# ShuhongChen/panic3d-anime-reconstruction

Hardware: AMD Instinct MI355X
Metric: rendered rays/sec at 512^2 img x 96 samples/ray (higher is better)
Workload: dtype f32

## Files before the change

### panic3d-anime-reconstruction_amd/_build.py

```python
import os
import subprocess

HERE = os.path.dirname(os.path.abspath(__file__))
CSRC = os.path.join(HERE, "csrc")
SO = os.path.join(HERE, "libpanic3d_hip.so")
SOURCES = ["p3d_kernels.hip", "p3d_synthesis.hip", "p3d_conv_plain.hip", "p3d_conv_up.hip", "p3d_conv_up4.hip", "p3d_fir.hip", "p3d_torgb.hip",
           "p3d_mcubes.hip", "p3d_paste.hip", "p3d_render_grad.hip", "p3d_synthesis_grad.hip"]
HEADERS = ["p3d_math.hpp", "p3d_decode.hpp", "p3d_lds_layout.hpp", "p3d_render_plan.hpp", "p3d_conv_common.hpp", "p3d_conv_plan.hpp", "p3d_conv_stage.hpp", os.path.join("..", "..", "include", "panic3d_hip.h"),
           os.path.join("..", "..", "include", "p3d_numerics.h"), os.path.join("..", "..", "include", "p3d_mc_table.h"),
           "p3d_decode_grad.hpp", os.path.join("..", "..", "include", "p3d_render_grad.h"),
           os.path.join("..", "..", "include", "p3d_synthesis_grad.h")]
HIPCC_FLAGS = ["--offload-arch=gfx950", "-O3", "-std=c++17", "-ffp-contract=off", "-fno-fast-math", "-fno-slp-vectorize",
               "-mllvm", "-pragma-unroll-threshold=200000", "-fPIC", "-shared"]


def _hipcc():
    for c in (os.environ.get("HIPCC"), "/opt/rocm/bin/hipcc", "hipcc"):
        if c and (os.path.sep not in c or os.path.exists(c)):
            return c
    raise RuntimeError("hipcc not found")


def source_hash():
    import hashlib
    h = hashlib.sha256()
    for s in sorted(SOURCES + HEADERS):
        with open(os.path.join(CSRC, s), "rb") as f:
            h.update(s.encode() + b"\0" + f.read())
    return h.hexdigest()[:16]


RENDER_UNIT = ["p3d_kernels.hip", "p3d_decode.hpp", "p3d_lds_layout.hpp", "p3d_render_plan.hpp", "p3d_math.hpp", os.path.join("..", "..", "include", "panic3d_hip.h"),
               os.path.join("..", "..", "include", "p3d_numerics.h")]


def render_source_hash():
    import hashlib
    h = hashlib.sha256()
    for s in sorted(RENDER_UNIT):
        with open(os.path.join(CSRC, s), "rb") as f:
            h.update(s.encode() + b"\0" + f.read())
    return h.hexdigest()[:16]


SYNTHESIS_UNIT = ["p3d_synthesis.hip", "p3d_conv_plain.hip", "p3d_conv_up.hip", "p3d_conv_up4.hip", "p3d_fir.hip", "p3d_torgb.hip", "p3d_conv_common.hpp",
                  "p3d_conv_plan.hpp", "p3d_conv_stage.hpp", os.path.join("..", "..", "include", "panic3d_hip.h")]


def synthesis_source_hash():
    import hashlib
    h = hashlib.sha256()
    for s in sorted(SYNTHESIS_UNIT):
        with open(os.path.join(CSRC, s), "rb") as f:
            h.update(s.encode() + b"\0" + f.read())
    return h.hexdigest()[:16]


def built_hash(so=SO):
    import re
    try:
        with open(so, "rb") as f:
            m = re.search(rb"libpanic3d_hip gfx950[^\0]{0,64}src=([0-9a-f]{16})", f.read())
    except OSError:
        return None
    return m.group(1).decode() if m else None
# ... 86 lines not shown
```

### panic3d-anime-reconstruction_amd/csrc/p3d_kernels.hip

```cpp
#include <hip/hip_runtime.h>
#include <stddef.h>
#include <stdlib.h>
#include <string.h>

#include <atomic>
#include <type_traits>

#include "p3d_decode.hpp"
#include "p3d_render_plan.hpp"

#define P3D_WAVES_PER_WG 4
#define P3D_WG (64 * P3D_WAVES_PER_WG)

__global__ __launch_bounds__(256) void k_planes_to_nhwc(const float* __restrict__ src, float* __restrict__ dst, int HW) {
    __shared__ float tile[32][65];
    const int p0 = blockIdx.x * 64;
    const size_t img = (size_t)blockIdx.y * 32 * HW;
    {
        int px = threadIdx.x & 63, c0 = threadIdx.x >> 6;
#pragma unroll
        for (int k = 0; k < 8; ++k) {
            int c = c0 + 4 * k;
            tile[c][px] = (p0 + px < HW) ? src[img + (size_t)c * HW + p0 + px] : 0.0f;
        }
    }
    __syncthreads();
    {
        int c = threadIdx.x & 31, q0 = threadIdx.x >> 5;
#pragma unroll
        for (int k = 0; k < 8; ++k) {
            int px = q0 + 8 * k;
            if (p0 + px < HW) dst[img + (size_t)(p0 + px) * 32 + c] = tile[c][px];
        }
    }
}

struct DecodeParams {
    const float* planes;
    const float* coords;
    const float *w0, *b0, *w1, *b1;
    float* out_sigma;
    float* out_rgb;
// ... 203 lines not shown
    P3dDecodeCfg cfg;
};

struct MarchState {
    double Td;
    float W, D;
    float prev_t, prev_sigma;
};

P3D_DEV uint32_t p3d_fmix32(uint32_t h) {
    h ^= h >> 16; h *= 0x85EBCA6Bu; h ^= h >> 13; h *= 0xC2B2AE35u; h ^= h >> 16;
    return h;
}
P3D_DEV float p3d_draw(uint32_t seed_lo, uint32_t seed_hi, uint32_t stream, size_t ray, int idx) {
    uint32_t h = p3d_fmix32(seed_lo ^ ((uint32_t)ray * 0x9E3779B1u));
    h = p3d_fmix32(h ^ seed_hi ^ ((uint32_t)((unsigned long long)ray >> 32) * 0x7FEB352Du) ^ (((uint32_t)idx * 2u + stream) * 0x846CA68Bu));
    return (float)(h >> 8) * 0x1p-24f;
}

P3D_DEV float p3d_march_weight(MarchState& st, float t, float sigma, float& tm_out) {
    float dl = t - st.prev_t;
    float sm = (st.prev_sigma + sigma) * 0.5f;
    float tm = (st.prev_t + t) * 0.5f;
    float rho = p3d_softplus(sm - 1.0f);
    float dd = rho * dl;
    float alpha = 1.0f - p3d_exp(-dd);
    float T = (float)st.Td;
    float w = alpha * T;
    st.Td = st.Td * (double)((1.0f - alpha) + 1e-10f);
    tm_out = tm;
    return w;
}

P3D_DEV constexpr int p3d_pow2_ceil(int n) { int p = 1; while (p < n) p <<= 1; return p; }
template <int NR>
P3D_DEV void p3d_sort_network(float (&a)[NR]) {
    constexpr int N = p3d_pow2_ceil(NR);
#pragma unroll
    for (int pp = 1; pp < N; pp <<= 1) {
#pragma unroll
        for (int k = pp; k >= 1; k >>= 1) {
#pragma unroll
            for (int jj = k % pp; jj + k < N; jj += 2 * k) {
#pragma unroll
                for (int i = 0; i < k; ++i) {
                    if (i + jj + k < NR && (i + jj) / (2 * pp) == (i + jj + k) / (2 * pp)) {
                        float x = a[i + jj], y = a[i + jj + k];
                        a[i + jj] = __builtin_fminf(x, y);
                        a[i + jj + k] = __builtin_fmaxf(x, y);
                    }
                }
            }
        }
    }
}

template <int RS = 32>
P3D_DEV void p3d_lds_insertion_sort(float* A, int n, int j) {
    for (int i = 1; i < n; ++i) {
        float key = A[i * RS + j];
        int q = i - 1;
        while (q >= 0) {
            float v = A[q * RS + j];
            if (!(v > key)) break;
            A[(q + 1) * RS + j] = v;
            --q;
        }
        A[(q + 1) * RS + j] = key;
    }
}

template <int B, int RS, typename TCF>
P3D_DEV void p3d_inverse_cdf(const float* cdfA, TCF tc, int Ns, int j, const float (&ui)[B], float (&out)[B], int (&k_out)[B]) {
    const int n = Ns + 1;
    int pos[B];
#pragma unroll
    for (int q = 0; q < B; ++q) pos[q] = 0;
#pragma unroll
    for (int step = 128; step >= 1; step >>= 1) {
        if (step <= n) {
            float c[B];
#pragma unroll
            for (int q = 0; q < B; ++q) c[q] = cdfA[((pos[q] + step <= n) ? pos[q] + step - 1 : 0) * RS + j];
#pragma unroll
            for (int q = 0; q < B; ++q) pos[q] = ((pos[q] + step <= n) && (c[q] <= ui[q])) ? pos[q] + step : pos[q];
        }
    }
    float cb[B], ca[B], t0[B], t1[B], t2[B], t3[B];
#pragma unroll
    for (int q = 0; q < B; ++q) {
        const int k = pos[q], below = k - 1 > 0 ? k - 1 : 0, above = k < Ns ? k : Ns;
        k_out[q] = k;
        cb[q] = cdfA[below * RS + j]; ca[q] = cdfA[above * RS + j];
        t0[q] = tc(below); t1[q] = tc(below + 1);
        t2[q] = tc(above); t3[q] = tc(above + 1);
    }
#pragma unroll
    for (int q = 0; q < B; ++q) {
        float den = ca[q] - cb[q];
        if (den < 1e-5f) den = 1.0f;
        const float bb = 0.5f * (t0[q] + t1[q]), ba = 0.5f * (t2[q] + t3[q]);
        out[q] = bb + ((ui[q] - cb[q]) / den) * (ba - bb);
        asm volatile("" : "+v"(out[q]));
    }
}

#define P3D_NF_EXACT(NF) ((NF) == 48 || (NF) == 96)
template <int NF, bool DUMP, bool FAST, bool EARLY, bool TCG = p3d_render_tcg(NF, DUMP, EARLY)>
__global__ __launch_bounds__(64 * P3D_RENDER_WAVES, p3d_render_occ(NF, TCG)) void k_render(RenderParams p) {
    static_assert(!(DUMP && EARLY), "dumps need every sample decoded");
    static_assert(!TCG || p3d_render_tcg(NF, DUMP, EARLY), "TCG exists only for the production 96-key kernel");
    extern __shared__ __attribute__((aligned(16))) float lds[];
    p3d_load_mlp_to_lds(lds, p.w0, p.b0, p.w1, p.b1, !FAST);
    if constexpr (FAST) p3d_load_mlp_f16_to_lds(lds, p.w0, p.w1);
    __syncthreads();
    const int lane = threadIdx.x & 63, wave = threadIdx.x >> 6, j = lane & 31, h = lane >> 5;
    long long nblk = gridDim.x, b = blockIdx.x;
    const long long swz = p.swz;
    long long full = (nblk / (8 * swz)) * (8 * swz);
    long long bs = b;
    if (b < full) {
        long long slot = b >> 3, x = b & 7;
        const long long g = slot / swz, xr = p.blocked ? ((x + g) & 7) : x;
        bs = g * (8 * swz) + xr * swz + (slot % swz);
    }
    const int nwaves = blockDim.x >> 6;
    long long tile = bs * nwaves + wave;
    if (tile >= p.ntiles) return;
    float* wl = lds + (FAST ? P3D_LDS_FAST_FLOATS : P3D_LDS_MLP_FLOATS) + 4 + (size_t)wave * p.lds_rows * 32;

    const int Sc = p.Sc, Sf = P3D_NF_EXACT(NF) ? NF : p.Sf, S = Sc + Sf;
    long long n = tile / p.tiles_per_img, tl = tile - n * p.tiles_per_img;
    long long r;
    if (p.tile_w > 0) {
        long long ty = tl / p.tiles_x, tx = tl - ty * p.tiles_x;
        if (p.blocked) {
            const long long st = tl >> 8;
            const int q = (int)(tl & 255), SX = p.tiles_x >> 4;
            tx = (st % SX) * 16 + (q & 15);
            ty = (st / SX) * 16 + (q >> 4);
        }
        const int lx = (j & 1) | ((j >> 1) & 6), ly = ((j >> 1) & 1) | ((j >> 3) & 2);
        r = (ty * 4 + ly) * p.tile_w + tx * 8 + lx;
    } else {
        r = tl * 32 + j;
    }
    const bool active = r < p.R;
    const long long rc = active ? r : p.R - 1;
    const size_t ray = (size_t)n * p.R + rc;

    P3dPlaneGeom g;
    g.halfW = 0.5f * (float)p.W; g.halfH = 0.5f * (float)p.H; g.fW = (float)p.W; g.fH = (float)p.H; g.W = p.W;
    g.plane_bytes = (uint32_t)p.H * (uint32_t)p.W * 128u;
    unsigned nlo = __builtin_amdgcn_readfirstlane((unsigned)n);
    const float* pbase = p.planes + ((p.cfg.flags & P3D_FLAG_SHARED_PLANES) ? (size_t)0 : (size_t)nlo * 3 * (g.plane_bytes / 4));
    auto rs = __builtin_amdgcn_make_buffer_rsrc((void*)pbase, 0, 3 * g.plane_bytes, 0x00020000);
    const P3dDecodeCfg cfg = p.cfg;
    constexpr bool early = EARLY;
    const bool f_crop = (cfg.flags & P3D_FLAG_CROP) != 0;
    int ndec = 0;

// ... 55 lines not shown
        for (int i0 = 0; i0 < Sc; i0 += 8) {
            float jv[8];
#pragma unroll
            for (int q = 0; q < 8; ++q) {
                const int iq = i0 + q < Sc ? i0 + q : Sc - 1;
                jv[q] = p.rng ? p3d_draw(p.seed_lo, p.seed_hi, 0u, ray, iq) : jit[iq];
            }
#pragma unroll
            for (int q = 0; q < 8; ++q) {
                const int i = i0 + q;
                if (i < Sc) {
                    float lin = (i < Sc / 2) ? p3d_fma(step, (float)i, p.ray_start) : p3d_fma(-step, (float)(Sc - 1 - i), p.ray_end);
                    float t = lin + jv[q] * p.depth_delta;
                    if (limits) {
                        const float prod = ((float)i / (float)(Sc - 1)) * span;
                        t = (rs + prod) + jv[q] * rdelta;
                    } else if (p.disparity) {
                        const float s01 = 1.0f / (float)(Sc - 1);
                        const float l01 = (i < Sc / 2) ? p3d_fma(s01, (float)i, 0.0f) : p3d_fma(-s01, (float)(Sc - 1 - i), 1.0f);
                        const float dd = l01 + jv[q] * p.depth_delta;
                        const float ta_ = p.ray_start * (1.0f - dd), tb_ = p.ray_end * dd;
                        t = 1.0f / (ta_ + tb_);
                    }
                    tcA[i * 32 + j] = t;
                    unsorted |= (t < prev);
                    prev = t;
                    tcmin = __builtin_fminf(tcmin, t);
                    tcmax = __builtin_fmaxf(tcmax, t);
                    if constexpr (DUMP) if (dump && p.dumps.depths_coarse) p.dumps.depths_coarse[ray * Sc + i] = t;
                }
            }
        }
    }
    float tmin = __builtin_inff(), tmax = -__builtin_inff();
    if (Sf > 0) {
        MarchState st;
        st.Td = 1.0; st.W = 0.0f; st.D = 0.0f; st.prev_t = 0.0f; st.prev_sigma = 0.0f;
        uint32_t mword = 0;
        if constexpr (TCG) {
            float prev = -__builtin_inff(), pmax = -__builtin_inff();
            for (int i0 = 0; i0 < Sc; i0 += 8) {
                float jv[8];
#pragma unroll
                for (int q = 0; q < 8; ++q) jv[q] = jit_at(i0 + q < Sc ? i0 + q : Sc - 1);
#pragma unroll
                for (int q = 0; q < 8; ++q) {
                    const int i = i0 + q;
                    if (i >= Sc) break;
                    const float t = depth_of(i, jv[q]);
                    unsorted |= (t < prev);
                    bad_order |= (t < pmax);
                    pmax = __builtin_fmaxf(pmax, prev);
                    prev = t;
                    tcmin = __builtin_fminf(tcmin, t);
                    tcmax = __builtin_fmaxf(tcmax, t);
                    const float px = ox + t * dx, py = oy + t * dy, pz = oz + t * dz;
                    float sigma = P3D_SIGMA_MASKED;
                    const bool cropped = f_crop && (__builtin_fabsf(px) > cfg.crop_limit || __builtin_fabsf(pz) > cfg.crop_limit);
                    const bool live = !(cropped || st.Td < 1e-60);
                    const bool skip = __builtin_amdgcn_ballot_w64(live) == 0;
                    if (!skip) {
                        f32x16 dummy;
                        p3d_decode_wave<false, true>(lds, rs, g, cfg, px, py, pz, sigma, dummy, live);
                    }
                    mword |= (cropped || (live && sigma == P3D_SIGMA_MASKED)) ? (1u << (i & 31)) : 0u;
                    if ((i & 31) == 31 || i == Sc - 1) {
// ... 7 lines not shown
                    st.prev_t = t; st.prev_sigma = sigma;
                    ndec += skip ? 0 : 1;
                }
            }
        } else
        for (int i = 0; i < Sc; ++i) {
            float t = tcA[i * 32 + j];
            float px = ox + t * dx, py = oy + t * dy, pz = oz + t * dz;
            float sigma = P3D_SIGMA_MASKED;
            bool skip = false, live = true, cropped = false;
            if (early) {
                cropped = f_crop && (__builtin_fabsf(px) > cfg.crop_limit || __builtin_fabsf(pz) > cfg.crop_limit);
                live = !(cropped || st.Td < 1e-60);
                skip = __builtin_amdgcn_ballot_w64(live) == 0;
            }
            if (!skip) {
                f32x16 dummy;
                p3d_decode_wave<false, true>(lds, rs, g, cfg, px, py, pz, sigma, dummy, live);
            }
            if (early) {
                mword |= (cropped || (live && sigma == P3D_SIGMA_MASKED)) ? (1u << (i & 31)) : 0u;
                if ((i & 31) == 31 || i == Sc - 1) { mkA[(i >> 5) * 32 + j] = mword; mword = 0; }
            }
            if constexpr (DUMP) if (dump && p.dumps.sigma_coarse) p.dumps.sigma_coarse[ray * Sc + i] = sigma;
            if (i > 0) {
                float tm;
                float w = p3d_march_weight(st, t, sigma, tm);
                wcA[(i - 1) * 32 + j] = w;
                if constexpr (DUMP) if (dump && p.dumps.weights_coarse) p.dumps.weights_coarse[ray * (Sc - 1) + i - 1] = w;
            }
            st.prev_t = t; st.prev_sigma = sigma;
            if constexpr (!DUMP) ndec += skip ? 0 : 1;
        }
        const int Ns = Sc - 3;
        {
            double sum = 0.0;
            float wa = wcA[0 * 32 + j], wb = wcA[1 * 32 + j];
            for (int jj = 0; jj < Ns; ++jj) {
                float wc = wcA[(jj + 2) * 32 + j];
                float m1 = __builtin_fmaxf(wa, wb), m2 = __builtin_fmaxf(wb, wc);
                float v = ((m1 + m2) * 0.5f + 0.01f) + 1e-5f;
                sum += (double)v;
                wcA[(jj + 1) * 32 + j] = v;
                wa = wb; wb = wc;
            }
            float fsum = (float)sum;
            double acc = 0.0;
            wcA[j] = 0.0f;
            for (int jj = 0; jj < Ns; ++jj) {
                float pdf = wcA[(jj + 1) * 32 + j] / fsum;
                acc += (double)pdf;
                wcA[(jj + 1) * 32 + j] = (float)acc;
            }
        }
        const float* uu = p.u + ray * Sf;
        constexpr int DB = 8;
        if constexpr (NF > 0) {
            float tf[NF];
#pragma unroll
            for (int i = 0; i < NF; ++i)
                tf[i] = (i < Sf) ? (p.rng ? p3d_draw(p.seed_lo, p.seed_hi, 1u, ray, i) : uu[i]) : 0.0f;
#pragma unroll
            for (int i0 = 0; i0 < NF; i0 += DB) {
                if (i0 < Sf) {
                    float ub[DB], vb[DB];
                    int kb[DB];
#pragma unroll
                    for (int q = 0; q < DB; ++q) ub[q] = tf[i0 + q];
                    if constexpr (TCG) p3d_inverse_cdf<DB, 32>(wcA, tc_raw, Ns, j, ub, vb, kb);
                    else p3d_inverse_cdf<DB, 32>(wcA, tc_lds, Ns, j, ub, vb, kb);
#pragma unroll
                    for (int q = 0; q < DB; ++q) {
                        tf[i0 + q] = (i0 + q < Sf) ? vb[q] : __builtin_inff();
                        if constexpr (DUMP) {
                            if (dump && i0 + q < Sf && p.dumps.depths_fine) p.dumps.depths_fine[ray * Sf + i0 + q] = vb[q];
                            if (dump && i0 + q < Sf && p.dumps.inds) p.dumps.inds[ray * Sf + i0 + q] = kb[q];
                        }
                    }
                } else {
#pragma unroll
                    for (int q = 0; q < DB; ++q) tf[i0 + q] = __builtin_inff();
                }
            }
            p3d_sort_network<NF>(tf);
#pragma unroll
            for (int i = 0; i < NF; ++i)
                if (i < Sf) {
                    tfA[i * 32 + j] = tf[i];
                    if constexpr (TCG) {
                        const float px = ox + tf[i] * dx, pz = oz + tf[i] * dz;
                        const uint32_t b = (f_crop && (__builtin_fabsf(px) > cfg.crop_limit || __builtin_fabsf(pz) > cfg.crop_limit)) ? (1u << (i & 31)) : 0u;
                        if (i < 32) fw0 |= b; else if (i < 64) fw1 |= b; else fw2 |= b;
                    }
                }
        } else {
            for (int i0 = 0; i0 < Sf; i0 += DB) {
                float ub[DB], vb[DB];
                int kb[DB];
#pragma unroll
                for (int q = 0; q < DB; ++q) {
                    const int iq = i0 + q < Sf ? i0 + q : Sf - 1;
                    ub[q] = p.rng ? p3d_draw(p.seed_lo, p.seed_hi, 1u, ray, iq) : uu[iq];
                }
                p3d_inverse_cdf<DB, 32>(wcA, tc_lds, Ns, j, ub, vb, kb);
#pragma unroll
                for (int q = 0; q < DB; ++q) {
                    if (i0 + q < Sf) {
                        tfA[(i0 + q) * 32 + j] = vb[q];
                        if constexpr (DUMP) {
                            if (dump && p.dumps.depths_fine) p.dumps.depths_fine[ray * Sf + i0 + q] = vb[q];
                            if (dump && p.dumps.inds) p.dumps.inds[ray * Sf + i0 + q] = kb[q];
                        }
                    }
                }
            }
            p3d_lds_insertion_sort(tfA, Sf, j);
        }
        if constexpr (TCG) {
            wave_unsorted = __builtin_amdgcn_ballot_w64(unsorted) != 0;
            wave_bad = __builtin_amdgcn_ballot_w64(bad_order) != 0;
            if (wave_unsorted) { mw0 = 0u; mw1 = 0u; mw2 = 0u; }
        } else
        if (__builtin_amdgcn_ballot_w64(unsorted) != 0) {
            p3d_lds_insertion_sort(tcA, Sc, j);
            if (early) {
                for (int i = 0; i < ((Sc + 31) >> 5); ++i) mkA[i * 32 + j] = 0u;
            }
        }
    }
    MarchState st;
    st.Td = 1.0; st.W = 0.0f; st.D = 0.0f; st.prev_t = 0.0f; st.prev_sigma = 0.0f;
    f32x16 C, prev_rgb;
    float Cx = 0.0f, Cy = 0.0f, Cz = 0.0f;
#pragma unroll
    for (int c = 0; c < 16; ++c) { C[c] = 0.0f; prev_rgb[c] = 0.0f; }
    {
        int ci = 0, fi = 0;
        float ta = TCG ? 0.0f : tcA[j], tb = (Sf > 0) ? tfA[j] : __builtin_inff();
        tmin = __builtin_fminf(tcmin, tb);
        tmax = __builtin_fmaxf(tcmax, (Sf > 0) ? tfA[(Sf - 1) * 32 + j] : -__builtin_inff());
        bool prev_skipped = false, first = true, done = false;
        int m = 0;
        auto is_cropped = [&](float t) {
            const float px = ox + t * dx, pz = oz + t * dz;
            return f_crop && (__builtin_fabsf(px) > cfg.crop_limit || __builtin_fabsf(pz) > cfg.crop_limit);
        };
        auto advance = [&](bool take_c) {
            ci += take_c ? 1 : 0;
            fi += take_c ? 0 : 1;
            const int cq = ci < Sc ? ci : Sc - 1, fq = fi < Sf ? fi : (Sf > 0 ? Sf - 1 : 0);
            const float nv = (take_c ? tcA : tfA)[(take_c ? cq : fq) * 32 + j];
            ta = take_c ? nv : ta;
            tb = take_c ? tb : nv;
        };
        float tcn = 0.0f;
        if constexpr (TCG) {
            uint32_t slw[6], knw[6];
#pragma unroll
            for (int w = 0; w < 6; ++w) { slw[w] = 0u; knw[w] = 0u; }
            for (int i0 = 0; i0 < Sc; i0 += 8) {
                float tv[8];
                int pos[8];
#pragma unroll
                for (int q = 0; q < 8; ++q) { tv[q] = tc_sorted(i0 + q < Sc ? i0 + q : Sc - 1); pos[q] = 0; }
#pragma unroll
                for (int step = 64; step >= 1; step >>= 1) {
                    float c[8];
#pragma unroll
                    for (int q = 0; q < 8; ++q) c[q] = tfA[((pos[q] + step <= Sf) ? pos[q] + step - 1 : 0) * 32 + j];
#pragma unroll
                    for (int q = 0; q < 8; ++q) pos[q] = ((pos[q] + step <= Sf) && (c[q] < tv[q])) ? pos[q] + step : pos[q];
                }
#pragma unroll
                for (int q = 0; q < 8; ++q) {
                    const int i = i0 + q;
                    if (i >= Sc) break;
                    const uint32_t mwv = (i < 32) ? mw0 : (i < 64 ? mw1 : mw2);
                    const bool known = is_cropped(tv[q]) || ((mwv >> (i & 31)) & 1u);
                    const int P = i + pos[q], pw = P >> 5;
                    const uint32_t b = 1u << (P & 31);
#pragma unroll
                    for (int w = 0; w < 6; ++w) {
                        slw[w] |= (pw == w) ? b : 0u;
                        knw[w] |= (pw == w && known) ? b : 0u;
                    }
                }
            }
            if (__builtin_amdgcn_ballot_w64((fw0 | fw1 | fw2) != 0u) != 0) {
                int fk = 0;
#pragma unroll
                for (int w = 0; w < 6; ++w) {
                    if (w * 32 < S) {
                        uint32_t kk = 0u;
                        for (int b = 0; b < 32; ++b) {
                            const bool isf = !((slw[w] >> b) & 1u) && (w * 32 + b < S);
                            const uint32_t fwv = (fk < 32) ? fw0 : (fk < 64 ? fw1 : fw2);
                            kk |= (isf && ((fwv >> (fk & 31)) & 1u)) ? (1u << b) : 0u;
                            fk += isf ? 1 : 0;
                        }
                        knw[w] |= kk;
                    }
                }
            }
#pragma unroll
            for (int w = 0; w < 6; ++w)
                if (w < nmw) { knA[w * 32 + j] = knw[w]; slA[w * 32 + j] = slw[w]; }
            tcn = tc_sorted(0);
        } else
        if constexpr (EARLY) {
            uint32_t kw = 0u, sw = 0u;
            for (int q = 0; q < S; ++q) {
                const bool take_c = (ci < Sc) && (fi >= Sf || ta <= tb);
                bool known = is_cropped(take_c ? ta : tb);
                if (take_c && Sf > 0) known = known || ((mkA[(ci >> 5) * 32 + j] >> (ci & 31)) & 1u);
                kw |= known ? (1u << (q & 31)) : 0u;
                sw |= take_c ? (1u << (q & 31)) : 0u;
                advance(take_c);
                if ((q & 31) == 31 || q == S - 1) {
                    knA[(q >> 5) * 32 + j] = kw; slA[(q >> 5) * 32 + j] = sw;
                    kw = 0u; sw = 0u;
                }
            }
            ci = 0;
        }
        for (int it = 0;; ++it) {
            bool take_c, known = false;
            float t;
            if constexpr (!EARLY) {
                if (it >= S) break;
                take_c = (ci < Sc) && (fi >= Sf || ta <= tb);
                t = take_c ? ta : tb;
                advance(take_c);
            } else {
                if (!done && st.Td < (FAST ? 2e-6 : 1e-60)) done = true;
                if (!done && (first || st.prev_sigma <= 602.0f)) {
                    bool any = false, last_c = false;
                    while (m < S) {
                        const int sh = m & 31, left = (32 - sh < S - m) ? 32 - sh : S - m;
                        const uint32_t kw = knA[(m >> 5) * 32 + j] >> sh, sw = slA[(m >> 5) * 32 + j] >> sh;
                        int run = (~kw != 0u) ? __builtin_ctz(~kw) : 32;
                        run = run < left ? run : left;
                        if (run > 0) {
                            const uint32_t inrun = run >= 32 ? 0xffffffffu : ((1u << run) - 1u);
                            ci += __builtin_popcount(sw & inrun);
                            last_c = (sw >> (run - 1)) & 1u;
                            any = true;
                            m += run;
                        }
                        if (run < left) break;
                    }
                    if (any) {
                        if constexpr (TCG) {
                            const float pc = tc_sorted(ci > 0 ? ci - 1 : 0);
                            tcn = tc_sorted(ci < Sc ? ci : Sc - 1);
                            st.prev_t = last_c ? pc : tfA[(m - ci - 1 > 0 ? m - ci - 1 : 0) * 32 + j];
                        } else
                        st.prev_t = last_c ? tcA[(ci - 1) * 32 + j] : tfA[(m - ci - 1) * 32 + j];
                        st.prev_sigma = P3D_SIGMA_MASKED;
                        prev_skipped = true; first = false;
                    }
                    done = m >= S;
                }
                if (__builtin_amdgcn_ballot_w64(!done) == 0) break;
                const int mm = done ? S - 1 : m;
                const uint32_t kb = knA[(mm >> 5) * 32 + j] >> (mm & 31), sb = slA[(mm >> 5) * 32 + j] >> (mm & 31);
                take_c = (sb & 1u) != 0u;
                known = !done && (kb & 1u) != 0u;
                const int cq = ci < Sc ? ci : Sc - 1, fq = (m - ci < Sf) ? m - ci : (Sf > 0 ? Sf - 1 : 0);
                if constexpr (TCG) t = take_c ? tcn : tfA[fq * 32 + j];
                else t = (take_c || Sf == 0) ? tcA[cq * 32 + j] : tfA[fq * 32 + j];
                if (!done) { ++m; ci += take_c ? 1 : 0; }
                if constexpr (TCG) {
                    if (!done && take_c) tcn = tc_sorted(ci < Sc ? ci : Sc - 1);
                }
            }
            const bool have = EARLY ? !done : true;
            const float px = ox + t * dx, py = oy + t * dy, pz = oz + t * dz;
            float sigma = P3D_SIGMA_MASKED;
            f32x16 rgb;
#pragma unroll
            for (int c = 0; c < 16; ++c) rgb[c] = 0.0f;
            const bool live = have && !known;
            bool skipped = true;
            if (__builtin_amdgcn_ballot_w64(live) != 0) {
                bool have_rgb;
                if constexpr (FAST) have_rgb = p3d_decode_wave_fast<true, true, EARLY, true>(lds, rs, g, cfg, px, py, pz, sigma, rgb, live);
                else have_rgb = p3d_decode_wave<true, true, EARLY>(lds, rs, g, cfg, px, py, pz, sigma, rgb, live);
                if constexpr (!DUMP) ndec += 1;
                skipped = !live || !have_rgb;
                if (known) sigma = P3D_SIGMA_MASKED;
            }
            if constexpr (DUMP) {
                if (dump && p.dumps.depths_sorted) p.dumps.depths_sorted[ray * S + m] = t;
                if (dump && p.dumps.sigma_sorted) p.dumps.sigma_sorted[ray * S + m] = sigma;
            }
            const bool marching = have && !first;
            float w = 0.0f, tm = 0.0f;
            if (marching) w = p3d_march_weight(st, t, sigma, tm);
            const float ppx = ox + st.prev_t * dx, ppy = oy + st.prev_t * dy, ppz = oz + st.prev_t * dz;
            if (early) {
                if (__builtin_amdgcn_ballot_w64(marching && prev_skipped && w != 0.0f) != 0) {
                    float s2;
                    f32x16 c2;
                    if constexpr (FAST) p3d_decode_wave_fast<true, true>(lds, rs, g, cfg, ppx, ppy, ppz, s2, c2);
                    else p3d_decode_wave<true>(lds, rs, g, cfg, ppx, ppy, ppz, s2, c2);
                    if (prev_skipped) prev_rgb = c2;
                    prev_skipped = false;
                }
                if (__builtin_amdgcn_ballot_w64(marching && skipped && w != 0.0f) != 0) {
                    float s2;
                    if constexpr (FAST) p3d_decode_wave_fast<true, true>(lds, rs, g, cfg, px, py, pz, s2, rgb);
                    else p3d_decode_wave<true>(lds, rs, g, cfg, px, py, pz, s2, rgb);
                    skipped = false;
                }
            }
            if (have) {
                if (!first) {
#pragma unroll
                    for (int c = 0; c < 16; ++c) C[c] = p3d_fma(w, (prev_rgb[c] + rgb[c]) * 0.5f, C[c]);
                    Cx = p3d_fma(w, (ppx + px) * 0.5f, Cx);
                    Cy = p3d_fma(w, (ppy + py) * 0.5f, Cy);
                    Cz = p3d_fma(w, (ppz + pz) * 0.5f, Cz);
                    st.W = st.W + w;
                    st.D = p3d_fma(w, tm, st.D);
                }
                st.prev_t = t; st.prev_sigma = sigma;
                prev_rgb = rgb;
                prev_skipped = skipped;
                first = false;
                if constexpr (!EARLY) ++m;
            }
        }
    }
    {
        const float Wt = st.W;
        float d = st.D / Wt;
        if (d != d) d = __builtin_inff();
#pragma unroll
        for (int c = 0; c < 16; ++c) {
            float v = C[c];
            if (p.white_back) v = (v + 1.0f) - Wt;
            C[c] = v * 2.0f - 1.0f;
        }
        if (p.white_back) { Cx = (Cx + 1.0f) - Wt; Cy = (Cy + 1.0f) - Wt; Cz = (Cz + 1.0f) - Wt; }
        Cx = Cx * 2.0f - 1.0f; Cy = Cy * 2.0f - 1.0f; Cz = Cz * 2.0f - 1.0f;
        if (active) {
            float* dst = p.out_feat + ray * 32 + 4 * h;
#pragma unroll
            for (int q = 0; q < 4; ++q) *(f32x4*)(dst + 8 * q) = (f32x4){C[4 * q], C[4 * q + 1], C[4 * q + 2], C[4 * q + 3]};
            if (h == 0) {
                p.out_depth[ray] = d;
                p.out_wsum[ray] = Wt;
                p.out_xyz[ray * 3] = Cx; p.out_xyz[ray * 3 + 1] = Cy; p.out_xyz[ray * 3 + 2] = Cz;
                if constexpr (DUMP) if (p.dumps.depth_unclamped) p.dumps.depth_unclamped[ray] = st.D / Wt;
            }
        }
    }
    if (!active) { tmin = __builtin_inff(); tmax = -__builtin_inff(); }
#pragma unroll
    for (int o = 32; o >= 1; o >>= 1) {
        tmin = __builtin_fminf(tmin, __shfl_xor(tmin, o));
        tmax = __builtin_fmaxf(tmax, __shfl_xor(tmax, o));
    }
    if (lane == 0) {
        atomicMin(p.gminmax, p3d_f2ord(tmin));
        atomicMax(p.gminmax + 1, p3d_f2ord(tmax));
        if (p.per_view_clamp) {
            atomicMin(p.gminmax + 4 + 2 * nlo, p3d_f2ord(tmin));
            atomicMax(p.gminmax + 5 + 2 * nlo, p3d_f2ord(tmax));
        }
        if constexpr (!DUMP) atomicAdd((unsigned long long*)(p.gminmax + 2), (unsigned long long)ndec);
    }
}

template <int X>
P3D_DEV float p3d_lane_xor(float v) {
    return __builtin_bit_cast(float, __builtin_amdgcn_ds_swizzle(__builtin_bit_cast(int, v), 0x1f | (X << 10)));
}

template <int N>
P3D_DEV float p3d_select(const float (&x)[N], int k) {
    static_assert(N == 2 || N == 4, "two or four entries");
    const float x0 = x[0], x1 = x[1];
    if constexpr (N == 2) {
        return (k & 1) ? x1 : x0;
    } else {
        const float x2 = x[2], x3 = x[3];
        return (k & 2) ? ((k & 1) ? x3 : x2) : ((k & 1) ? x1 : x0);
    }
}

template <int SLOTS, int NF, bool FAST, bool WO = false>
__global__ __launch_bounds__(64 * P3D_RENDER_WAVES, p3d_render_slots_occ(SLOTS, FAST)) void k_render_slots(RenderParams p) {
    static_assert(SLOTS == 2 || SLOTS == 4, "16 rays x 2 slots or 8 rays x 4 slots per wave");
    static_assert(!WO || (FAST && SLOTS == 4), "the weights-only launch exists for the tolerance mode (the renderer class's default, what the paste runs)");
    constexpr int RPW = 32 / SLOTS;
// ... 654 lines not shown
        e = p3d_ensure_dynamic_lds(k_decode_points<false, SV, FV>, lds_bytes);                                        \
        if (e == hipSuccess)                                                                                          \
            hipLaunchKernelGGL((k_decode_points<false, SV, FV>), dim3((unsigned)blocks), dim3(P3D_WG), lds_bytes, (hipStream_t)stream, p); \
    } while (0)
    if (staged) { if (fastd) P3D_LAUNCH_GRID(true, true); else P3D_LAUNCH_GRID(true, false); }
    else { if (fastd) P3D_LAUNCH_GRID(false, true); else P3D_LAUNCH_GRID(false, false); }
    if (e != hipSuccess) return (int)e;
    return p3d_check_launch();
}

int p3d_decode_features_f32(const float* feats, int N, int64_t M, const float* w0, const float* b0, const float* w1, const float* b1,
                            int force_sigmoid, float* out_sigma, float* out_rgb, void* stream) {
    if (!feats || !w0 || !b0 || !w1 || !b1 || !out_sigma || !out_rgb || N <= 0 || M <= 0) return P3D_E_ARG;
    if ((((uintptr_t)feats | (uintptr_t)out_rgb) & 15) != 0) return P3D_E_RANGE;
    DecodeFeatParams p;
    p.feats = feats; p.w0 = w0; p.b0 = b0; p.w1 = w1; p.b1 = b1; p.out_sigma = out_sigma; p.out_rgb = out_rgb;
    p.M = M; p.tiles_per_img = (M + 31) / 32; p.ntiles = p.tiles_per_img * N;
    memset(&p.cfg, 0, sizeof(p.cfg));
    p.cfg.flags = force_sigmoid ? P3D_FLAG_FORCE_SIGMOID : 0;
    const size_t lds_bytes = (size_t)(P3D_LDS_MLP_FLOATS + 4) * 4;
    long long blocks = (p.ntiles + P3D_WAVES_PER_WG - 1) / P3D_WAVES_PER_WG;
    if (blocks > 256 * 8) blocks = 256 * 8;
    hipError_t e = p3d_ensure_dynamic_lds(k_decode_features, lds_bytes);
    if (e != hipSuccess) return (int)e;
    hipLaunchKernelGGL(k_decode_features, dim3((unsigned)blocks), dim3(P3D_WG), lds_bytes, (hipStream_t)stream, p);
    return p3d_check_launch();
}

size_t p3d_render_workspace_bytes(int N, int64_t R, int Sc, int Sf) {
    (void)R; (void)Sc; (void)Sf;
    return p3d_render_plan_workspace_bytes(N);
}

int p3d_render_plan_info(int N, int64_t R, int ray_tile_w, const p3d_opts* opts, int has_dumps, int has_ray_limits, int64_t* out, int cap) {
    if (!opts) return P3D_E_ARG;
    const RenderPlan pl = p3d_render_plan(N, R, ray_tile_w, *opts, has_dumps != 0, has_ray_limits != 0);
    if (pl.err) return pl.err;
    if (!out || cap < 6) return P3D_E_ARG;
    const int64_t info[6] = {pl.slots, pl.ntiles, pl.decode_steps_full, pl.grid, pl.block, (int64_t)pl.lds_bytes};
    for (int i = 0; i < 6; ++i) out[i] = info[i];
    return P3D_OK;
}

int p3d_render_f32(const float* planes, int N, int H, int W, const float* rays_o, const float* rays_d, int64_t R,
                   int ray_tile_w, const float* jitter, const float* u, const float* w0, const float* b0,
                   const float* w1, const float* b1, const p3d_opts* opts, float* out_feat, float* out_depth,
                   float* out_wsum, float* out_xyz, void* workspace, size_t workspace_bytes, const p3d_dumps* dumps,
                   void* stream) {
    return p3d_render_limits_f32(planes, N, H, W, rays_o, rays_d, R, ray_tile_w, jitter, u, w0, b0, w1, b1, nullptr, nullptr, opts,
                                 out_feat, out_depth, out_wsum, out_xyz, workspace, workspace_bytes, dumps, stream);
}

static int render_impl(const float* planes, int N, int H, int W, const float* rays_o, const float* rays_d, int64_t R,
                       int ray_tile_w, const float* jitter, const float* u, int rng, uint64_t seed, const float* w0, const float* b0,
                       const float* w1, const float* b1, const float* ray_start, const float* ray_end, const p3d_opts* opts,
                       float* out_feat, float* out_depth, float* out_wsum, float* out_xyz, void* workspace,
                       size_t workspace_bytes, const p3d_dumps* dumps, void* stream);

int p3d_render_limits_f32(const float* planes, int N, int H, int W, const float* rays_o, const float* rays_d, int64_t R,
                          int ray_tile_w, const float* jitter, const float* u, const float* w0, const float* b0,
                          const float* w1, const float* b1, const float* ray_start, const float* ray_end, const p3d_opts* opts,
                          float* out_feat, float* out_depth, float* out_wsum, float* out_xyz, void* workspace,
                          size_t workspace_bytes, const p3d_dumps* dumps, void* stream) {
    return render_impl(planes, N, H, W, rays_o, rays_d, R, ray_tile_w, jitter, u, 0, 0, w0, b0, w1, b1, ray_start, ray_end, opts, out_feat,
                       out_depth, out_wsum, out_xyz, workspace, workspace_bytes, dumps, stream);
}
// ... 143 lines not shown
```

Baseline: 84.20 million.

## Split fine-sample sort and merge-bit construction across both wave halves

For the exact-NF path, each half-wave now draws and sorts only half of the fine samples and then combines them with a permlane32 swap exchange and a bitonic valley merge, instead of every lane sorting all NF samples. The coarse-rank bit construction in the TCG path and the early-termination merge-bit loop are likewise split between the two halves, with results combined through shuffles or LDS atomicOr. It also adds compile-time-gated phase timing instrumentation and moves the sort helpers into a shared header. The aim is to halve per-lane sort and merge register and ALU work, at the cost of extra cross-lane exchanges, fences and LDS atomics.

```diff
diff --git a/panic3d-anime-reconstruction_amd/_build.py b/panic3d-anime-reconstruction_amd/_build.py
--- a/panic3d-anime-reconstruction_amd/_build.py
+++ b/panic3d-anime-reconstruction_amd/_build.py
@@ -6,7 +6,7 @@
 SO = os.path.join(HERE, "libpanic3d_hip.so")
 SOURCES = ["p3d_kernels.hip", "p3d_synthesis.hip", "p3d_conv_plain.hip", "p3d_conv_up.hip", "p3d_conv_up4.hip", "p3d_fir.hip", "p3d_torgb.hip",
            "p3d_mcubes.hip", "p3d_paste.hip", "p3d_render_grad.hip", "p3d_synthesis_grad.hip"]
-HEADERS = ["p3d_math.hpp", "p3d_decode.hpp", "p3d_lds_layout.hpp", "p3d_render_plan.hpp", "p3d_conv_common.hpp", "p3d_conv_plan.hpp", "p3d_conv_stage.hpp", os.path.join("..", "..", "include", "panic3d_hip.h"),
+HEADERS = ["p3d_math.hpp", "p3d_decode.hpp", "p3d_lds_layout.hpp", "p3d_render_plan.hpp", "p3d_phase_timing.hpp", "p3d_importance.hpp", "p3d_conv_common.hpp", "p3d_conv_plan.hpp", "p3d_conv_stage.hpp", os.path.join("..", "..", "include", "panic3d_hip.h"),
            os.path.join("..", "..", "include", "p3d_numerics.h"), os.path.join("..", "..", "include", "p3d_mc_table.h"),
            "p3d_decode_grad.hpp", os.path.join("..", "..", "include", "p3d_render_grad.h"),
            os.path.join("..", "..", "include", "p3d_synthesis_grad.h")]
@@ -30,7 +30,7 @@
     return h.hexdigest()[:16]
 
 
-RENDER_UNIT = ["p3d_kernels.hip", "p3d_decode.hpp", "p3d_lds_layout.hpp", "p3d_render_plan.hpp", "p3d_math.hpp", os.path.join("..", "..", "include", "panic3d_hip.h"),
+RENDER_UNIT = ["p3d_kernels.hip", "p3d_decode.hpp", "p3d_lds_layout.hpp", "p3d_render_plan.hpp", "p3d_phase_timing.hpp", "p3d_importance.hpp", "p3d_math.hpp", os.path.join("..", "..", "include", "panic3d_hip.h"),
                os.path.join("..", "..", "include", "p3d_numerics.h")]
 
 
diff --git a/panic3d-anime-reconstruction_amd/csrc/p3d_importance.hpp b/panic3d-anime-reconstruction_amd/csrc/p3d_importance.hpp
--- /dev/null
+++ b/panic3d-anime-reconstruction_amd/csrc/p3d_importance.hpp
@@ -0,0 +1,111 @@
+#pragma once
+
+#if defined(__HIPCC__)
+#define P3D_IMP_FN __host__ __device__ __forceinline__
+#define P3D_IMP_UNROLL _Pragma("unroll")
+#else
+#define P3D_IMP_FN inline
+#define P3D_IMP_UNROLL
+#endif
+
+struct P3dFloatKey {
+    P3D_IMP_FN static float mn(float a, float b) { return __builtin_fminf(a, b); }
+    P3D_IMP_FN static float mx(float a, float b) { return __builtin_fmaxf(a, b); }
+    P3D_IMP_FN static float neg(float a) { return -a; }
+};
+
+P3D_IMP_FN constexpr int p3d_pow2_ceil(int n) { int p = 1; while (p < n) p <<= 1; return p; }
+
+template <int NR, typename K = P3dFloatKey, typename T>
+P3D_IMP_FN void p3d_sort_merge_pass(T (&a)[NR], int pp) {
+    constexpr int N = p3d_pow2_ceil(NR);
+P3D_IMP_UNROLL
+    for (int k = pp; k >= 1; k >>= 1) {
+P3D_IMP_UNROLL
+        for (int jj = k % pp; jj + k < N; jj += 2 * k) {
+P3D_IMP_UNROLL
+            for (int i = 0; i < k; ++i) {
+                if (i + jj + k < NR && (i + jj) / (2 * pp) == (i + jj + k) / (2 * pp)) {
+                    T x = a[i + jj], y = a[i + jj + k];
+                    a[i + jj] = K::mn(x, y);
+                    a[i + jj + k] = K::mx(x, y);
+                }
+            }
+        }
+    }
+}
+template <int NR, typename K = P3dFloatKey, typename T>
+P3D_IMP_FN void p3d_sort_network(T (&a)[NR]) {
+P3D_IMP_UNROLL
+    for (int pp = 1; pp < p3d_pow2_ceil(NR); pp <<= 1) p3d_sort_merge_pass<NR, K>(a, pp);
+}
+
+template <typename K = P3dFloatKey, typename T>
+P3D_IMP_FN void p3d_cross_half_exchange(T lo, T hi_neg, T& lo_out_neg, T& hi_out) {
+    lo_out_neg = K::mx(K::neg(lo), hi_neg);
+    hi_out = K::mx(lo, K::neg(hi_neg));
+}
+
+template <int H, typename K = P3dFloatKey, typename T>
+P3D_IMP_FN void p3d_valley_merge(T (&a)[H]) {
+    constexpr int N = p3d_pow2_ceil(H);
+P3D_IMP_UNROLL
+    for (int k = N / 2; k >= 1; k >>= 1) {
+P3D_IMP_UNROLL
+        for (int i = 0; i < H; ++i) {
+            if ((i & k) == 0 && i + k < H) {
+                T x = a[i], y = a[i + k];
+                a[i] = K::mn(x, y);
+                a[i + k] = K::mx(x, y);
+            }
+        }
+    }
+}
+
+P3D_IMP_FN constexpr int p3d_half_rank(int H, int h, int i) { return h ? H + i : H - 1 - i; }
+
+P3D_IMP_FN int p3d_merge_split_steps(int Sc, int Sf) {
+    int n = Sc < Sf ? Sc : Sf, s = 0;
+    while (n > 0) { ++s; n >>= 1; }
+    return s;
+}
+template <typename RD>
+P3D_IMP_FN int p3d_merge_split(RD rd, int Sc, int Sf, int D, int steps) {
+    int lo = D - Sf > 0 ? D - Sf : 0, hi = D < Sc ? D : Sc;
+    for (int s = 0; s < steps; ++s) {
+        const int mid = (lo + hi) >> 1;
+        const int cm = mid < Sc - 1 ? mid : Sc - 1, fm = D - mid - 1 < 0 ? 0 : (D - mid - 1 < Sf ? D - mid - 1 : Sf - 1);
+        const bool behind = rd(false, fm) < rd(true, cm);
+        const bool open = lo < hi;
+        hi = (open && behind) ? mid : hi;
+        lo = (open && !behind) ? mid + 1 : lo;
+    }
+    return lo;
+}
+
+template <typename RD, typename KN, typename PUT>
+P3D_IMP_FN void p3d_merge_bits_half(RD rd, KN known, PUT put, int Sc, int Sf, int h) {
+    const int S = Sc + Sf, D = S >> 1, qb = h ? D : 0, qe = h ? S : D;
+    int ci = p3d_merge_split(rd, Sc, Sf, qb, p3d_merge_split_steps(Sc, Sf)), fi = qb - ci;
+    const float inf = __builtin_inff();
+    float ta = rd(true, ci < Sc ? ci : Sc - 1), tb = Sf > 0 ? rd(false, fi < Sf ? fi : Sf - 1) : inf;
+    unsigned kw = 0u, sw = 0u;
+    for (int it = 0; it < S - D; ++it) {
+        const int q = qb + it;
+        const bool mine = q < qe;
+        const bool take_c = (ci < Sc) && (fi >= Sf || ta <= tb);
+        const bool kn = known(take_c, take_c ? ci : fi, take_c ? ta : tb);
+        kw |= (mine && kn) ? (1u << (q & 31)) : 0u;
+        sw |= (mine && take_c) ? (1u << (q & 31)) : 0u;
+        ci += take_c ? 1 : 0;
+        fi += take_c ? 0 : 1;
+        const int cq = ci < Sc ? ci : Sc - 1, fq = fi < Sf ? fi : (Sf > 0 ? Sf - 1 : 0);
+        const float nv = rd(take_c, take_c ? cq : fq);
+        ta = take_c ? nv : ta;
+        tb = take_c ? tb : nv;
+        if (mine && ((q & 31) == 31 || q == qe - 1)) {
+            put(q >> 5, kw, sw);
+            kw = 0u; sw = 0u;
+        }
+    }
+}
diff --git a/panic3d-anime-reconstruction_amd/csrc/p3d_kernels.hip b/panic3d-anime-reconstruction_amd/csrc/p3d_kernels.hip
--- a/panic3d-anime-reconstruction_amd/csrc/p3d_kernels.hip
+++ b/panic3d-anime-reconstruction_amd/csrc/p3d_kernels.hip
@@ -8,6 +8,8 @@
 
 #include "p3d_decode.hpp"
 #include "p3d_render_plan.hpp"
+#include "p3d_phase_timing.hpp"
+#include "p3d_importance.hpp"
 
 #define P3D_WAVES_PER_WG 4
 #define P3D_WG (64 * P3D_WAVES_PER_WG)
@@ -277,29 +279,6 @@
     return w;
 }
 
-P3D_DEV constexpr int p3d_pow2_ceil(int n) { int p = 1; while (p < n) p <<= 1; return p; }
-template <int NR>
-P3D_DEV void p3d_sort_network(float (&a)[NR]) {
-    constexpr int N = p3d_pow2_ceil(NR);
-#pragma unroll
-    for (int pp = 1; pp < N; pp <<= 1) {
-#pragma unroll
-        for (int k = pp; k >= 1; k >>= 1) {
-#pragma unroll
-            for (int jj = k % pp; jj + k < N; jj += 2 * k) {
-#pragma unroll
-                for (int i = 0; i < k; ++i) {
-                    if (i + jj + k < NR && (i + jj) / (2 * pp) == (i + jj + k) / (2 * pp)) {
-                        float x = a[i + jj], y = a[i + jj + k];
-                        a[i + jj] = __builtin_fminf(x, y);
-                        a[i + jj + k] = __builtin_fmaxf(x, y);
-                    }
-                }
-            }
-        }
-    }
-}
-
 template <int RS = 32>
 P3D_DEV void p3d_lds_insertion_sort(float* A, int n, int j) {
     for (int i = 1; i < n; ++i) {
@@ -356,6 +335,7 @@
     static_assert(!(DUMP && EARLY), "dumps need every sample decoded");
     static_assert(!TCG || p3d_render_tcg(NF, DUMP, EARLY), "TCG exists only for the production 96-key kernel");
     extern __shared__ __attribute__((aligned(16))) float lds[];
+    P3D_PHASE_START();
     p3d_load_mlp_to_lds(lds, p.w0, p.b0, p.w1, p.b1, !FAST);
     if constexpr (FAST) p3d_load_mlp_f16_to_lds(lds, p.w0, p.w1);
     __syncthreads();
@@ -372,6 +352,7 @@
     const int nwaves = blockDim.x >> 6;
     long long tile = bs * nwaves + wave;
     if (tile >= p.ntiles) return;
+    P3D_PHASE(P3D_PH_WEIGHTS);
     float* wl = lds + (FAST ? P3D_LDS_FAST_FLOATS : P3D_LDS_MLP_FLOATS) + 4 + (size_t)wave * p.lds_rows * 32;
 
     const int Sc = p.Sc, Sf = P3D_NF_EXACT(NF) ? NF : p.Sf, S = Sc + Sf;
@@ -493,6 +474,7 @@
             }
         }
     }
+    P3D_PHASE(P3D_PH_STRAT);
     float tmin = __builtin_inff(), tmax = -__builtin_inff();
     if (Sf > 0) {
         MarchState st;
@@ -566,6 +548,7 @@
             st.prev_t = t; st.prev_sigma = sigma;
             if constexpr (!DUMP) ndec += skip ? 0 : 1;
         }
+        P3D_PHASE(P3D_PH_COARSE);
         const int Ns = Sc - 3;
         {
             double sum = 0.0;
@@ -587,9 +570,72 @@
                 wcA[(jj + 1) * 32 + j] = (float)acc;
             }
         }
+        P3D_PHASE(P3D_PH_CDF);
         const float* uu = p.u + ray * Sf;
         constexpr int DB = 8;
-        if constexpr (NF > 0) {
+        if constexpr (P3D_NF_EXACT(NF)) {
+            typedef uint32_t u32x2 __attribute__((ext_vector_type(2)));
+            constexpr int H = NF / 2;
+            static_assert(H % DB == 0, "whole batches of draws per half");
+            const int d0 = h * H;
+            const uint32_t neg1 = h ? 0x80000000u : 0u, neg0 = h ? 0u : 0x80000000u;
+            float tf[H];
+#pragma unroll
+            for (int i = 0; i < H; ++i)
+                tf[i] = p.rng ? p3d_draw(p.seed_lo, p.seed_hi, 1u, ray, d0 + i) : uu[d0 + i];
+#pragma unroll
+            for (int i0 = 0; i0 < H; i0 += DB) {
+                float ub[DB], vb[DB];
+                int kb[DB];
+#pragma unroll
+                for (int q = 0; q < DB; ++q) ub[q] = tf[i0 + q];
+                if constexpr (TCG) p3d_inverse_cdf<DB, 32>(wcA, tc_raw, Ns, j, ub, vb, kb);
+                else p3d_inverse_cdf<DB, 32>(wcA, tc_lds, Ns, j, ub, vb, kb);
+#pragma unroll
+                for (int q = 0; q < DB; ++q) {
+                    tf[i0 + q] = vb[q];
+                    if constexpr (DUMP) {
+                        if (active && p.dumps.depths_fine) p.dumps.depths_fine[ray * Sf + d0 + i0 + q] = vb[q];
+                        if (active && p.dumps.inds) p.dumps.inds[ray * Sf + d0 + i0 + q] = kb[q];
+                    }
+                }
+            }
+            P3D_PHASE(P3D_PH_DRAWS);
+#pragma unroll
+            for (int i = 0; i < H; ++i) tf[i] = __builtin_bit_cast(float, __builtin_bit_cast(uint32_t, tf[i]) ^ neg1);
+            p3d_sort_network<H>(tf);
+#pragma unroll
+            for (int i = 0; i < H; i += 2) {
+                u32x2 in = __builtin_amdgcn_permlane32_swap(__builtin_bit_cast(uint32_t, tf[i]), __builtin_bit_cast(uint32_t, tf[i + 1]), false, false);
+                const uint32_t in0 = in.x, in1 = in.y;
+                float mn_neg, mx;
+                p3d_cross_half_exchange(__builtin_bit_cast(float, in0), __builtin_bit_cast(float, in1), mn_neg, mx);
+                u32x2 out = __builtin_amdgcn_permlane32_swap(__builtin_bit_cast(uint32_t, mn_neg), __builtin_bit_cast(uint32_t, mx), false, false);
+                const uint32_t out0 = out.x, out1 = out.y;
+                tf[i] = __builtin_bit_cast(float, out0);
+                tf[i + 1] = __builtin_bit_cast(float, out1);
+            }
+            p3d_valley_merge<H>(tf);
+            __builtin_amdgcn_fence(__ATOMIC_ACQ_REL, "wavefront");
+            const int row0 = p3d_half_rank(H, h, 0), rstep = h ? 1 : -1;
+            uint64_t crop = 0ull;
+#pragma unroll
+            for (int i = 0; i < H; ++i) {
+                const float v = __builtin_bit_cast(float, __builtin_bit_cast(uint32_t, tf[i]) ^ neg0);
+                tfA[(row0 + rstep * i) * 32 + j] = v;
+                if constexpr (TCG) {
+                    const float px = ox + v * dx, pz = oz + v * dz;
+                    crop |= (f_crop && (__builtin_fabsf(px) > cfg.crop_limit || __builtin_fabsf(pz) > cfg.crop_limit)) ? (1ull << i) : 0ull;
+                }
+            }
+            __builtin_amdgcn_fence(__ATOMIC_ACQ_REL, "wavefront");
+            if constexpr (TCG) {
+                static_assert(H >= 32 && H < 64, "the 96 rank bits as 64 + 32");
+                const uint64_t g0 = h ? (crop << H) : (__builtin_bitreverse64(crop) >> (64 - H));
+                fw0 = (uint32_t)g0; fw1 = (uint32_t)(g0 >> 32); fw2 = h ? (uint32_t)(crop >> (64 - H)) : 0u;
+                fw0 |= __shfl_xor(fw0, 32); fw1 |= __shfl_xor(fw1, 32); fw2 |= __shfl_xor(fw2, 32);
+            }
+        } else if constexpr (NF > 0) {
             float tf[NF];
 #pragma unroll
             for (int i = 0; i < NF; ++i)
@@ -616,6 +662,7 @@
                     for (int q = 0; q < DB; ++q) tf[i0 + q] = __builtin_inff();
                 }
             }
+            P3D_PHASE(P3D_PH_DRAWS);
             p3d_sort_network<NF>(tf);
 #pragma unroll
             for (int i = 0; i < NF; ++i)
@@ -648,8 +695,10 @@
                     }
                 }
             }
+            P3D_PHASE(P3D_PH_DRAWS);
             p3d_lds_insertion_sort(tfA, Sf, j);
         }
+        P3D_PHASE(P3D_PH_SORT);
         if constexpr (TCG) {
             wave_unsorted = __builtin_amdgcn_ballot_w64(unsorted) != 0;
             wave_bad = __builtin_amdgcn_ballot_w64(bad_order) != 0;
@@ -692,11 +741,12 @@
             uint32_t slw[6], knw[6];
 #pragma unroll
             for (int w = 0; w < 6; ++w) { slw[w] = 0u; knw[w] = 0u; }
-            for (int i0 = 0; i0 < Sc; i0 += 8) {
+            const int Sch = ((Sc + 15) >> 4) << 3, ib = h * Sch;
+            for (int i0 = 0; i0 < Sch; i0 += 8) {
                 float tv[8];
                 int pos[8];
 #pragma unroll
-                for (int q = 0; q < 8; ++q) { tv[q] = tc_sorted(i0 + q < Sc ? i0 + q : Sc - 1); pos[q] = 0; }
+                for (int q = 0; q < 8; ++q) { tv[q] = tc_sorted(ib + i0 + q < Sc ? ib + i0 + q : Sc - 1); pos[q] = 0; }
 #pragma unroll
                 for (int step = 64; step >= 1; step >>= 1) {
                     float c[8];
@@ -707,11 +757,10 @@
                 }
 #pragma unroll
                 for (int q = 0; q < 8; ++q) {
-                    const int i = i0 + q;
-                    if (i >= Sc) break;
+                    const int i = ib + i0 + q;
                     const uint32_t mwv = (i < 32) ? mw0 : (i < 64 ? mw1 : mw2);
                     const bool known = is_cropped(tv[q]) || ((mwv >> (i & 31)) & 1u);
-                    const int P = i + pos[q], pw = P >> 5;
+                    const int P = i + pos[q], pw = (i < Sc) ? (P >> 5) : -1;
                     const uint32_t b = 1u << (P & 31);
 #pragma unroll
                     for (int w = 0; w < 6; ++w) {
@@ -720,6 +769,8 @@
                     }
                 }
             }
+#pragma unroll
+            for (int w = 0; w < 6; ++w) { slw[w] |= __shfl_xor(slw[w], 32); knw[w] |= __shfl_xor(knw[w], 32); }
             if (__builtin_amdgcn_ballot_w64((fw0 | fw1 | fw2) != 0u) != 0) {
                 int fk = 0;
 #pragma unroll
@@ -742,21 +793,21 @@
             tcn = tc_sorted(0);
         } else
         if constexpr (EARLY) {
-            uint32_t kw = 0u, sw = 0u;
-            for (int q = 0; q < S; ++q) {
-                const bool take_c = (ci < Sc) && (fi >= Sf || ta <= tb);
-                bool known = is_cropped(take_c ? ta : tb);
-                if (take_c && Sf > 0) known = known || ((mkA[(ci >> 5) * 32 + j] >> (ci & 31)) & 1u);
-                kw |= known ? (1u << (q & 31)) : 0u;
-                sw |= take_c ? (1u << (q & 31)) : 0u;
-                advance(take_c);
-                if ((q & 31) == 31 || q == S - 1) {
-                    knA[(q >> 5) * 32 + j] = kw; slA[(q >> 5) * 32 + j] = sw;
-                    kw = 0u; sw = 0u;
-                }
-            }
+            for (int w = 0; w < nmw; ++w) { knA[w * 32 + j] = 0u; slA[w * 32 + j] = 0u; }
+            __builtin_amdgcn_fence(__ATOMIC_ACQ_REL, "wavefront");
+            p3d_merge_bits_half(
+                [&](bool c, int i) { return (c ? tcA : tfA)[i * 32 + j]; },
+                [&](bool c, int i, float t) {
+                    bool known = is_cropped(t);
+                    if (c && Sf > 0) known = known || ((mkA[(i >> 5) * 32 + j] >> (i & 31)) & 1u);
+                    return known;
+                },
+                [&](int w, uint32_t kw, uint32_t sw) { atomicOr(&knA[w * 32 + j], kw); atomicOr(&slA[w * 32 + j], sw); },
+                Sc, Sf, h);
+            __builtin_amdgcn_fence(__ATOMIC_ACQ_REL, "wavefront");
             ci = 0;
         }
+        P3D_PHASE(P3D_PH_MERGE);
         for (int it = 0;; ++it) {
             bool take_c, known = false;
             float t;
@@ -808,6 +859,7 @@
                     if (!done && take_c) tcn = tc_sorted(ci < Sc ? ci : Sc - 1);
                 }
             }
+            P3D_PHASE(P3D_PH_SELECT);
             const bool have = EARLY ? !done : true;
             const float px = ox + t * dx, py = oy + t * dy, pz = oz + t * dz;
             float sigma = P3D_SIGMA_MASKED;
@@ -824,6 +876,7 @@
                 skipped = !live || !have_rgb;
                 if (known) sigma = P3D_SIGMA_MASKED;
             }
+            P3D_PHASE(P3D_PH_DECODE);
             if constexpr (DUMP) {
                 if (dump && p.dumps.depths_sorted) p.dumps.depths_sorted[ray * S + m] = t;
                 if (dump && p.dumps.sigma_sorted) p.dumps.sigma_sorted[ray * S + m] = sigma;
@@ -864,6 +917,7 @@
                 first = false;
                 if constexpr (!EARLY) ++m;
             }
+            P3D_PHASE(P3D_PH_MARCH);
         }
     }
     {
@@ -896,6 +950,8 @@
         tmin = __builtin_fminf(tmin, __shfl_xor(tmin, o));
         tmax = __builtin_fmaxf(tmax, __shfl_xor(tmax, o));
     }
+    P3D_PHASE(P3D_PH_OUT);
+    P3D_PHASE_FLUSH();
     if (lane == 0) {
         atomicMin(p.gminmax, p3d_f2ord(tmin));
         atomicMax(p.gminmax + 1, p3d_f2ord(tmax));
@@ -1616,6 +1672,18 @@
     return p3d_render_plan_workspace_bytes(N);
 }
 
+#ifdef P3D_PHASE_TIMING
+int p3d_phase_read(unsigned long long* out, int n, int reset) {
+    unsigned long long v[P3D_PH_N];
+    if (hipDeviceSynchronize() != hipSuccess || hipMemcpyFromSymbol(v, HIP_SYMBOL(g_p3d_phase), sizeof(v)) != hipSuccess) return -1;
+    for (int q = 0; q < n && q < P3D_PH_N; ++q) out[q] = v[q];
+    if (reset) {
+        memset(v, 0, sizeof(v));
+        if (hipMemcpyToSymbol(HIP_SYMBOL(g_p3d_phase), v, sizeof(v)) != hipSuccess) return -1;
+    }
+    return P3D_PH_N;
+}
+#endif
 int p3d_render_plan_info(int N, int64_t R, int ray_tile_w, const p3d_opts* opts, int has_dumps, int has_ray_limits, int64_t* out, int cap) {
     if (!opts) return P3D_E_ARG;
     const RenderPlan pl = p3d_render_plan(N, R, ray_tile_w, *opts, has_dumps != 0, has_ray_limits != 0);
diff --git a/panic3d-anime-reconstruction_amd/csrc/p3d_phase_timing.hpp b/panic3d-anime-reconstruction_amd/csrc/p3d_phase_timing.hpp
--- /dev/null
+++ b/panic3d-anime-reconstruction_amd/csrc/p3d_phase_timing.hpp
@@ -0,0 +1,57 @@
+#pragma once
+
+#ifdef P3D_PHASE_TIMING
+enum P3dPhase {
+    P3D_PH_WEIGHTS = 0,
+    P3D_PH_STRAT,
+    P3D_PH_COARSE,
+    P3D_PH_CDF,
+    P3D_PH_DRAWS,
+    P3D_PH_SORT,
+    P3D_PH_MERGE,
+    P3D_PH_SELECT,
+    P3D_PH_DECODE,
+    P3D_PH_MARCH,
+    P3D_PH_OUT,
+    P3D_PH_WAVES,
+    P3D_PH_LIFE,
+    P3D_PH_N
+};
+__device__ unsigned long long g_p3d_phase[P3D_PH_N];
+
+struct P3dPhaseClock {
+    unsigned long long first, last, acc[P3D_PH_N];
+    __device__ __forceinline__ static unsigned long long now() {
+        unsigned long long t;
+        __builtin_amdgcn_sched_barrier(0);
+        asm volatile("s_memtime %0\n\ts_waitcnt lgkmcnt(0)" : "=s"(t) :: "memory");
+        __builtin_amdgcn_sched_barrier(0);
+        return t;
+    }
+    __device__ __forceinline__ void start() {
+#pragma unroll
+        for (int q = 0; q < P3D_PH_N; ++q) acc[q] = 0ull;
+        first = last = now();
+    }
+    __device__ __forceinline__ void mark(int slot) {
+        const unsigned long long t = now();
+        acc[slot] += t - last;
+        last = t;
+    }
+    __device__ __forceinline__ void flush() {
+        acc[P3D_PH_WAVES] = 1ull;
+        acc[P3D_PH_LIFE] = last - first;
+        if ((threadIdx.x & 63) == 0) {
+#pragma unroll
+            for (int q = 0; q < P3D_PH_N; ++q) atomicAdd(&g_p3d_phase[q], acc[q]);
+        }
+    }
+};
+#define P3D_PHASE_START() P3dPhaseClock p3d_phase_clock; p3d_phase_clock.start()
+#define P3D_PHASE(slot) p3d_phase_clock.mark(slot)
+#define P3D_PHASE_FLUSH() p3d_phase_clock.flush()
+#else
+#define P3D_PHASE_START() ((void)0)
+#define P3D_PHASE(slot) ((void)0)
+#define P3D_PHASE_FLUSH() ((void)0)
+#endif
```

New measurement: 86.27 million (median of 6 runs). +2.5%, better.
